# jiali-ms/JLM

Measured on AMD Instinct MI355X. Metric: decoded chars/sec at beam=10, vocab=50k (kana strings in -> n-best strings out, SURVEY 8d), higher is better.
Workload: dtype f32 (matrix products as 3-pass split-f16 MFMA, f32 accumulate; the vocabulary projection as f16 hi.hi + both cross terms in one block-scaled FP6 instruction per 32 k-values: f32-grade error, tests/test_gpu_kernels.py; scores f64; parity bars: step logits <= 1e-4 relative, 1-best identical, path scor

## Files before the change

__graft_entry__.py:

```python
import os
import subprocess
import sys

REPO = os.path.dirname(os.path.abspath(__file__))
CSRC = os.path.join(REPO, "jlm_amd", "csrc")
HIP_SOURCES = ["jlm_gemm.hip", "jlm_beam.hip", "jlm_split.hip", "jlm_gate.hip", "jlm_gate_p2.hip", "jlm_mixed.hip", "jlm_decode.hip", "jlm_score.hip", "jlm_topk.hip", "jlm_kmeans.hip", "jlm_train.hip"]
HOST_SOURCES = ["jlm_lattice.cpp"]


def _stale(target, sources):
    if not os.path.exists(target):
        return True
    t = os.path.getmtime(target)
    import glob
    deps = list(sources) + glob.glob(os.path.join(CSRC, "*.h")) + glob.glob(os.path.join(REPO, "include", "*.h"))
    return any(os.path.exists(s) and os.path.getmtime(s) > t for s in deps)


def _hipcc_accepts(hipcc, flags):
    key = (hipcc, tuple(flags))
    if key not in _hipcc_accepts.cache:
        import tempfile
        with tempfile.TemporaryDirectory() as d:
            src = os.path.join(d, "probe.hip")
            with open(src, "w") as f:
                f.write("__global__ void probe_kernel(float *p) { p[0] = 1.0f; }\n")
            rc = subprocess.call([hipcc, "--offload-arch=gfx950", "-c", "--cuda-device-only", "-o", os.path.join(d, "probe.o")] + list(flags) + [src],
                                 stdout=subprocess.DEVNULL, stderr=subprocess.DEVNULL)
        _hipcc_accepts.cache[key] = rc == 0
    return _hipcc_accepts.cache[key]


_hipcc_accepts.cache = {}


def build(force=False):
    hipcc = os.environ.get("HIPCC", "/opt/rocm/bin/hipcc")
    out = os.path.join(CSRC, "libjlm_hip.so")
    srcs = [os.path.join(CSRC, s) for s in HIP_SOURCES]
    if not _hipcc_accepts(hipcc, ["-mllvm", "-amdgpu-mfma-vgpr-form"]):
        raise RuntimeError("this hipcc does not accept -mllvm -amdgpu-mfma-vgpr-form: jlm_gate_ws.hip / jlm_mixed_w.hip cannot be built "
                           "correctly without it (their inline-asm loads into accumulation registers are not tracked by the compiler)")
    vgpr_form = ["-mllvm", "-amdgpu-mfma-vgpr-form"]
    no_nan = ["-fno-honor-nans", "-mno-amdgpu-ieee"]
    flagged = {"jlm_gate_ws.hip": vgpr_form, "jlm_mixed_w.hip": vgpr_form, "jlm_mx6.hip": no_nan + ["-fno-slp-vectorize"], "jlm_mx6w.hip": vgpr_form + no_nan,
               "jlm_frame_tail.hip": ["-fno-slp-vectorize"]}
    srcs = srcs + [os.path.join(CSRC, f) for f in flagged]
    if force or _stale(out, srcs):
        procs, objs = [], []
        for src in srcs:
            obj = src[:-4] + ".o"
            objs.append(obj)
            if force or _stale(obj, [src]):
                procs.append((src, subprocess.Popen([hipcc, "--offload-arch=gfx950", "-O3", "-std=c++17", "-fPIC", "-c", "-o", obj] +
                                                    flagged.get(os.path.basename(src), []) + [src], cwd=CSRC)))
        for src, pr in procs:
            if pr.wait() != 0:
                raise subprocess.CalledProcessError(pr.returncode, "hipcc -c " + src)
        subprocess.check_call([hipcc, "--offload-arch=gfx950", "-fPIC", "-shared", "-o", out] + objs, cwd=CSRC)
    host_srcs = [os.path.join(CSRC, s) for s in HOST_SOURCES if os.path.exists(os.path.join(CSRC, s))]
    if host_srcs:
        hout = os.path.join(CSRC, "libjlm_host.so")
        if force or _stale(hout, host_srcs):
            subprocess.check_call(["g++", "-O3", "-std=c++17", "-fPIC", "-shared", "-pthread", "-o", hout] + host_srcs,
                                  cwd=CSRC)
    rsrc = os.path.join(CSRC, "jlm_readout.c")
    rout = os.path.join(REPO, "jlm_amd", "_readout.so")
    if force or _stale(rout, [rsrc]):
        import sysconfig
        subprocess.check_call(["gcc", "-O2", "-fPIC", "-shared", "-I" + sysconfig.get_paths()["include"], "-o", rout, rsrc],
                              cwd=CSRC)
    tsrc = os.path.join(CSRC, "jlm_torch_ops.cpp")
    tout = os.path.join(REPO, "jlm_amd", "_torch_ops.so")
    if force or _stale(tout, [tsrc, out]):
        import torch
        from torch.utils import cpp_extension as ce
        tlib = ce.library_paths()[0]
        cmd = ["g++", "-O2", "-std=c++17", "-fPIC", "-shared", "-D__HIP_PLATFORM_AMD__", "-DUSE_ROCM",
               "-D_GLIBCXX_USE_CXX11_ABI=%d" % int(torch._C._GLIBCXX_USE_CXX11_ABI)]
        cmd += ["-I" + p for p in ce.include_paths()] + ["-I/opt/rocm/include", tsrc, "-o", tout, "-L" + tlib, "-ltorch", "-ltorch_cpu",
                                                         "-lc10", "-lc10_hip", "-ltorch_hip", "-L" + CSRC, "-ljlm_hip",
                                                         "-Wl,-rpath,$ORIGIN/csrc", "-Wl,-rpath," + tlib]
        subprocess.check_call(cmd, cwd=CSRC)
    if REPO not in sys.path:
        sys.path.insert(0, REPO)
    import jlm_amd
    from jlm_amd import _readout
    from jlm_amd import _lib, ops
    _lib.lib()
    ops.backend()
    from oracle import jlm_oracle


def smoke():
    import tempfile
    import numpy as np
    build()
    import torch
    assert torch.cuda.is_available(), "smoke() needs a GPU"
    from jlm_amd import config as jconfig, ops, synth
    assert type(ops.backend()).__name__ == "HipOps", "smoke() checks the HIP path (jlm_amd.ops.set_backend is a test hook)"
    from jlm_amd.decoder import Decoder
    from jlm_amd.decoder_dynamic import DynamicDecoder
    from oracle import jlm_oracle as orc
    root = tempfile.mkdtemp(prefix="jlm_smoke_")
    _cfg, _lex, _rd, alphabet = synth.build_fixture(root, "wide-vtable")
    jconfig.set_root(root)
    sents = synth.make_ragged_sentences(6, 3, 12, seed=42, alphabet=alphabet)
    score_atol = lambda s: 1e-6 * (len(s) + 1) + 2e-6
    dec = Decoder(1)
    assert dec.model.dev.mixed_idx == [0, 1, 2] or os.environ.get("JLM_LSE_MIXED") == "0" or os.environ.get("JLM_PRECISION") == "f32"
    got = dec.decode_batch(sents, beam_width=5)
    ref = orc.OracleDecoder(root, 1)
    for s, g in zip(sents, got):
        want = ref.decode(s, beam_width=5)
        assert [w for _, w in g][0] == [w for _, w in want][0], (s, g[0], want[0])
        np.testing.assert_allclose([x for x, _ in g], [x for x, _ in want], rtol=0, atol=score_atol(s))
    root2 = tempfile.mkdtemp(prefix="jlm_smoke_")
    synth.build_fixture(root2, "small-tied")
    jconfig.set_root(root2)
    dd = DynamicDecoder(1)
    got = dd.decode_batch(sents, beam_width=5, vocab_select=True)
    ref = orc.OracleDynamicDecoder(root2, 1)
    for s, g in zip(sents, got):
        want = ref.decode(s, beam_width=5, vocab_select=True)
        assert [w for _, w in g][0] == [w for _, w in want][0], (s, g[0], want[0])
        np.testing.assert_allclose([x for x, _ in g], [x for x, _ in want], rtol=0, atol=score_atol(s))
    print("smoke ok: static (D-softmax*) and dynamic decode match the oracle on", len(sents), "sentences")


if __name__ == "__main__":
    build(force="--force" in sys.argv)
    if "--smoke" in sys.argv:
        smoke()
```

jlm_amd/csrc/jlm_beam.hip:

```cpp
#include "jlm_common.h"
#include <type_traits>
#include <stdlib.h>

#define WL_THREADS 256
#define WL_ROWS 16

template <int MODE>
__global__ __launch_bounds__(WL_THREADS) void wordlist_kernel(
    SegTable segs, const float *__restrict__ b2, const float *__restrict__ T, int ldt,
    const int *__restrict__ g0v, const int *__restrict__ cnt, const int *__restrict__ cnt_idx,
    const int *__restrict__ wl, const int *__restrict__ wl_w, const int *__restrict__ wl_off, const int *__restrict__ wl_idx,
    int wl_base, const int *__restrict__ wl_out, float *__restrict__ edge, float *__restrict__ run_max,
    double *__restrict__ run_sum, double *__restrict__ lse, int merge, int beam) {
    extern __shared__ __attribute__((aligned(16))) float sm[];
    const int j = blockIdx.x;
    const int nrows = min(cnt[cnt_idx[j]], beam);
    if (nrows <= 0) return;
    const int gbase = g0v[j];
    const int lid = wl_base + wl_idx[j];
    const int w0 = wl_off[lid], nw = wl_off[lid + 1] - w0;
    if (MODE == 0 && nw == 0) return;
    const int tid = threadIdx.x;
    float *red = sm + (size_t)WL_ROWS * ldt;
    const int sub = tid & 7, slot = tid >> 3;
// ... 91 lines not shown
                for (int off = 32; off >= 1; off >>= 1) {
                    float m2 = __shfl_xor(rm[r], off), s2 = __shfl_xor(rs[r], off);
                    lse_merge(rm[r], rs[r], m2, s2);
                }
            }
            const int wave = tid >> 6, lane = tid & 63;
            __syncthreads();
            if (lane == 0)
                for (int r = 0; r < WL_ROWS; ++r) {
                    red[(wave * WL_ROWS + r) * 2] = rm[r];
                    red[(wave * WL_ROWS + r) * 2 + 1] = rs[r];
                }
            __syncthreads();
            if (tid < WL_ROWS && rc + tid < nrows) {
                float m = red[tid * 2], s = red[tid * 2 + 1];
                for (int w2 = 1; w2 < WL_THREADS / 64; ++w2)
                    lse_merge(m, s, red[(w2 * WL_ROWS + tid) * 2], red[(w2 * WL_ROWS + tid) * 2 + 1]);
                const int g = gbase + rc + tid;
                double S = (double)s;
                float M = m;
                if (merge) {
                    const float pm = run_max[g];
                    const double ps = run_sum[g];
                    M = fmaxf(pm, m);
                    S = ps * exp((double)pm - (double)M) + (double)s * exp((double)m - (double)M);
                }
                run_max[g] = M;
                run_sum[g] = S;
                lse[g] = (double)M + log(S);
            }
        }
    }
}

static int seg_table(const jlm_segment *segs_host, int n_segs, SegTable &t) {
    if (n_segs < 1 || n_segs > JLM_MAX_SEGMENTS) return -1;
    t.n = n_segs;
    for (int i = 0; i < n_segs; ++i) {
        t.s[i] = segs_host[i];
        if (t.s[i].k % 4 || t.s[i].ldb % 4 || t.s[i].t_off % 4) return -1;
    }
    return 0;
}

static size_t wl_lds_bytes(int , int ldt) { return ((size_t)WL_ROWS * ldt + 4 * WL_ROWS * 2) * sizeof(float); }

extern "C" int jlm_edge_logits(const jlm_segment *segs_host, int n_segs, const float *b2, const float *T, int ldt,
                               const int *g0, const int *cnt, const int *cnt_idx, const int *wl, const int *wl_off,
                               const int *wl_idx, int wl_base, const int *wl_out, float *edge, int beam, int n_groups,
                               void *stream) {
    return jlm_edge_logits_perm(segs_host, n_segs, b2, T, ldt, g0, cnt, cnt_idx, wl, nullptr, wl_off, wl_idx, wl_base, wl_out,
                                edge, beam, n_groups, stream);
}

extern "C" int jlm_edge_logits_perm(const jlm_segment *segs_host, int n_segs, const float *b2, const float *T, int ldt,
                                    const int *g0, const int *cnt, const int *cnt_idx, const int *wl, const int *wl_w,
                                    const int *wl_off, const int *wl_idx, int wl_base, const int *wl_out, float *edge, int beam,
                                    int n_groups, void *stream) {
    SegTable t;
    if (seg_table(segs_host, n_segs, t) || ldt % 4) return -1;
    if (n_groups <= 0) return 0;
    size_t lds = wl_lds_bytes(beam, ldt);
    if (lds > 160 * 1024) return -1;
    static JlmLdsGrant grant;
    if (int rc = jlm_grant_lds(grant, reinterpret_cast<const void *>(wordlist_kernel<0>), (int)lds)) return rc;
    hipLaunchKernelGGL(wordlist_kernel<0>, dim3(n_groups), dim3(WL_THREADS), lds, (hipStream_t)stream, t, b2, T, ldt,
                       g0, cnt, cnt_idx, wl, wl_w, wl_off, wl_idx, wl_base, wl_out, edge, nullptr, nullptr, nullptr, 0, beam);
    JLM_LAUNCH_CHECK();
    return 0;
}

static bool wl_split_hosts(const jlm_segment &s, int ldt) {
    const int ns = (s.k + 15) / 16;
    return ns >= 1 && ns <= 16 && s.k % 4 == 0 && s.ldb % 16 == 0 && s.ldb >= ns * 16 && s.t_off % 4 == 0 && ldt % 4 == 0;
}

extern "C" int jlm_wordlist_lse_form(const jlm_segment *segs_host, int n_segs, const jlm_segment *split_seg, int has_wl_w, int ldt,
                                     int beam, int max_words) {
    if (split_seg && n_segs == 1 && !has_wl_w && beam <= 64 && max_words >= JLM_WL_SPLIT_MIN_WORDS &&
        max_words <= JLM_WL_SPLIT_MAX_WORDS && wl_split_hosts(*split_seg, ldt))
        return JLM_WL_SPLIT;
    SegTable t;
    if (seg_table(segs_host, n_segs, t) || ldt % 4) return -1;
    static int use_mfma = -1;
    if (use_mfma < 0) { const char *e = getenv("JLM_WORDLIST_MFMA"); use_mfma = e ? atoi(e) : 1; }
    if (!has_wl_w && use_mfma && n_segs == 1 && beam <= 64 && segs_host[0].k >= 1 && segs_host[0].k <= 256) return JLM_WL_MFMA;
    if (wl_lds_bytes(beam, ldt) > 160 * 1024) return -1;
    return JLM_WL_F32;
}

extern "C" int jlm_wordlist_merge_form(const jlm_segment *segs_host, int n_segs, const jlm_segment *split_seg, int ldt, int beam,
                                       int max_words) {
    if (split_seg && n_segs == 1 && beam <= 64 && max_words <= JLM_WL_MERGE_MAX_WORDS && wl_split_hosts(*split_seg, ldt))
        return JLM_WL_MERGE_SPLIT;
    return jlm_wordlist_lse_form(segs_host, n_segs, split_seg, 0, ldt, beam, max_words);
}

extern "C" int jlm_wordlist_lse_mfma(const jlm_segment *seg_host, const float *b2, const float *T, int ldt, const int *g0,
                                     const int *cnt, const int *cnt_idx, const int *wl, const int *wl_off,
                                     const int *wl_idx, int wl_base, float *run_max, double *run_sum, double *lse,
                                     int merge, int beam, int n_groups, void *stream);

extern "C" int jlm_wordlist_lse(const jlm_segment *segs_host, int n_segs, const float *b2, const float *T, int ldt,
                                const int *g0, const int *cnt, const int *cnt_idx, const int *wl, const int *wl_off,
                                const int *wl_idx, int wl_base, float *run_max, double *run_sum, double *lse, int merge,
                                int beam, int n_groups, void *stream) {
    return jlm_wordlist_lse_perm(segs_host, n_segs, b2, T, ldt, g0, cnt, cnt_idx, wl, nullptr, wl_off, wl_idx, wl_base, run_max,
                                 run_sum, lse, merge, beam, n_groups, stream);
}

extern "C" int jlm_wordlist_lse_perm(const jlm_segment *segs_host, int n_segs, const float *b2, const float *T, int ldt,
                                     const int *g0, const int *cnt, const int *cnt_idx, const int *wl, const int *wl_w,
                                     const int *wl_off, const int *wl_idx, int wl_base, float *run_max, double *run_sum,
                                     double *lse, int merge, int beam, int n_groups, void *stream) {
    SegTable t;
    if (seg_table(segs_host, n_segs, t) || ldt % 4) return -1;
    if (n_groups <= 0) return 0;
    const int form = jlm_wordlist_lse_form(segs_host, n_segs, nullptr, wl_w != nullptr, ldt, beam, 0);
    if (form < 0) return -1;
    if (form == JLM_WL_MFMA)
        return jlm_wordlist_lse_mfma(segs_host, b2, T, ldt, g0, cnt, cnt_idx, wl, wl_off, wl_idx, wl_base, run_max, run_sum,
                                     lse, merge, beam, n_groups, stream);
    const size_t lds = wl_lds_bytes(beam, ldt);
    static JlmLdsGrant grant;
    if (int rc = jlm_grant_lds(grant, reinterpret_cast<const void *>(wordlist_kernel<1>), (int)lds)) return rc;
    hipLaunchKernelGGL(wordlist_kernel<1>, dim3(n_groups), dim3(WL_THREADS), lds, (hipStream_t)stream, t, b2, T, ldt,
                       g0, cnt, cnt_idx, wl, wl_w, wl_off, wl_idx, wl_base, nullptr, nullptr, run_max, run_sum, lse, merge, beam);
    JLM_LAUNCH_CHECK();
    return 0;
}

template <int CTRL, int ROW_MASK>
__device__ __forceinline__ void argmin_dpp_step(double &v, int &i) {
    const int lo = __double2loint(v), hi = __double2hiint(v);
    const int lo2 = __builtin_amdgcn_update_dpp(lo, lo, CTRL, ROW_MASK, 0xf, false);
    const int hi2 = __builtin_amdgcn_update_dpp(hi, hi, CTRL, ROW_MASK, 0xf, false);
    const int i2 = __builtin_amdgcn_update_dpp(i, i, CTRL, ROW_MASK, 0xf, false);
    const double v2 = __hiloint2double(hi2, lo2);
    if (v2 < v || (v2 == v && i2 < i)) { v = v2; i = i2; }
}
__device__ __forceinline__ void wave_argmin(double &v, int &i) {
    argmin_dpp_step<0xB1, 0xf>(v, i);
    argmin_dpp_step<0x4E, 0xf>(v, i);
    argmin_dpp_step<0x141, 0xf>(v, i);
    argmin_dpp_step<0x140, 0xf>(v, i);
    argmin_dpp_step<0x142, 0xa>(v, i);
    argmin_dpp_step<0x143, 0xc>(v, i);
    const int lo = __builtin_amdgcn_readlane(__double2loint(v), 63);
    const int hi = __builtin_amdgcn_readlane(__double2hiint(v), 63);
    i = __builtin_amdgcn_readlane(i, 63);
    v = __hiloint2double(hi, lo);
}

template <int MODE>
__global__ __launch_bounds__(64, 8) void beam_step_kernel(jlm_lattice lat, jlm_beam_state st, int frame, int max_cands) {
    extern __shared__ __attribute__((aligned(16))) double keys[];
    const int s = blockIdx.x, lane = threadIdx.x;
    const int B = lat.n_sent, beam = lat.beam, rmax = B * beam;
    const int len = lat.sent_len[s];
    const int fs = frame * B + s;
    if (frame > len) { if (lane == 0) st.cnt[fs] = 0; return; }
    const int nb = lat.end_off[fs], ne = lat.end_off[fs + 1];
    const int gout = frame * rmax + s * beam;
    const double INF = __longlong_as_double(0x7ff0000000000000LL);
    double *Sarr = keys + max_cands;
    int *gp_of = reinterpret_cast<int *>(Sarr + (MODE == 2 ? lat.n_frames * beam : 0));
    double *lse_new = reinterpret_cast<double *>(gp_of + ((max_cands + 1) & ~1));
    int *cnt_s = reinterpret_cast<int *>(lse_new + beam);
    double *win_v = reinterpret_cast<double *>(cnt_s + ((lat.n_frames + 1) & ~1));
    int *win_i = reinterpret_cast<int *>(win_v + beam);
    int K;
    if (frame == 0) {
        K = 1;
    } else {
        const bool fused = MODE == 0 && st.lse_part != nullptr;
        const int fprev = (frame - 1) * B + s;
        for (int f = lane; f < frame; f += 64) cnt_s[f] = st.cnt[f * B + s];
        const int kprev = st.cnt[fprev];
        if (fused && kprev > 0) {
            const int base = st.live_base[fprev];
            const float2 *part = reinterpret_cast<const float2 *>(st.lse_part);
            const int sub = lane & 7;
            for (int r0 = 0; r0 < kprev; r0 += 8) {
                const int r = r0 + (lane >> 3);
                float m = JLM_NEG_BIG;
                double sm = 0.0;
                if (r < kprev)
                    for (int p = sub; p < st.n_parts; p += 8) {
                        const float2 v = part[(size_t)p * st.ld_part + base + r];
                        const float mm = fmaxf(m, v.x);
                        sm = sm * (double)expf(m - mm) + (double)v.y * (double)expf(v.x - mm);
                        m = mm;
                    }
#pragma unroll
                for (int off = 4; off >= 1; off >>= 1) {
                    const float m2 = __shfl_xor(m, off);
                    const double s2 = __shfl_xor(sm, off);
                    const float mm = fmaxf(m, m2);
                    sm = sm * (double)expf(m - mm) + s2 * (double)expf(m2 - mm);
                    m = mm;
                }
                if (sub == 0 && r < kprev) {
                    double l = (double)m + log(sm);
                    if (!(fabs(l) < 1.0e300)) { if (st.flags) atomicOr(st.flags, 1); l = 1.0e30; }
                    lse_new[r] = l;
                    st.lse[(size_t)(frame - 1) * rmax + s * beam + r] = l;
                }
            }
        }
        const int C = (ne - nb) * beam;
        if (MODE == 2) {
            for (int f = 0; f < frame; ++f) {
                const int c = st.cnt[f * B + s];
                for (int l = lane; l < c; l += 64) {
                    const int g = f * rmax + s * beam + l;
                    const int p = st.bp[g];
                    double S = 0.0;
                    if (p >= 0) {
                        const int pf = p / rmax, pk = p - pf * rmax - s * beam;
                        S = Sarr[pf * beam + pk] + st.lse[p];
                    }
                    Sarr[f * beam + l] = S;
                }
                __syncthreads();
            }
        }
        __syncthreads();
        int nvalid = 0;
        double bv = INF;
        int bi = 0x7fffffff;
        constexpr int U = 4, NREG = 8;
        double kreg[NREG];
#pragma unroll
        for (int j = 0; j < NREG; ++j) kreg[j] = INF;
        auto group = [&](int it, auto REG0) {
            constexpr int reg0 = decltype(REG0)::value;
            const int c0 = lane + 64 * U * it;
            int n[U], k[U], sf[U];
#pragma unroll
            for (int u = 0; u < U; ++u) {
                const int c = min(c0 + 64 * u, C - 1);
                n[u] = nb + c / beam;
                k[u] = c % beam;
                sf[u] = lat.node_start[n[u]];
            }
            bool ok[U];
            double scv[U], lsv[U], ysv[U];
            float ev[U];
#pragma unroll
            for (int u = 0; u < U; ++u) {
                ok[u] = (c0 + 64 * u < C) && k[u] < cnt_s[sf[u]];
                const int gp = sf[u] * rmax + s * beam + (ok[u] ? k[u] : 0);
                ev[u] = st.edge[(size_t)n[u] * beam + k[u]];
                scv[u] = (MODE == 2) ? 0.0 : st.score[gp];
                lsv[u] = (MODE == 1) ? 0.0 : st.lse[gp];
                ysv[u] = (MODE == 2) ? st.ysum[gp] : 0.0;
                if (c0 + 64 * u < C) gp_of[c0 + 64 * u] = ok[u] ? gp : -1;
            }
#pragma unroll
            for (int u = 0; u < U; ++u) {
                const int c = c0 + 64 * u;
                if (c >= C) break;
                double sc = INF;
                if (ok[u]) {
                    const double e = (double)ev[u];
                    if (MODE == 0) sc = scv[u] + (((fused && sf[u] == frame - 1) ? lse_new[k[u]] : lsv[u]) - e);
                    else if (MODE == 1) sc = scv[u] - e;
                    else sc = (Sarr[sf[u] * beam + k[u]] + lsv[u]) - (ysv[u] + e);
                    ++nvalid;
                }
                if constexpr (reg0 >= 0) kreg[reg0 + u] = sc; else keys[c] = sc;
                if (sc < bv) { bv = sc; bi = c; }
            }
        };
        group(0, std::integral_constant<int, 0>{});
        if (C > 64 * U) group(1, std::integral_constant<int, U>{});
        for (int it = 2; 64 * U * it < C; ++it) group(it, std::integral_constant<int, -1>{});
#pragma unroll
        for (int off = 32; off >= 1; off >>= 1) nvalid += __shfl_xor(nvalid, off);
        K = min(beam, nvalid);
        for (int r = 0; r < K; ++r) {
            double v = bv;
            int i = bi;
            wave_argmin(v, i);
            if (lane == 0) { win_v[r] = v; win_i[r] = i; }
            if ((i & 63) == lane) {
                const int jw = i >> 6;
                if (jw >= NREG) keys[i] = INF;
                bv = INF;
                bi = 0x7fffffff;
#pragma unroll
                for (int j = 0; j < NREG; ++j) {
                    if (j == jw) kreg[j] = INF;
                    if (kreg[j] < bv) { bv = kreg[j]; bi = lane + 64 * j; }
                }
                for (int c = lane + 64 * NREG; c < C; c += 64) {
                    const double kv = keys[c];
                    if (kv < bv) { bv = kv; bi = c; }
                }
            }
        }
        __syncthreads();
    }
    for (int r = lane; r < K; r += 64) {
        const int g = gout + r;
        if (frame == 0) {
            st.score[g] = 0.0;
            if (st.ysum) st.ysum[g] = 0.0;
            st.bp[g] = -1;
            st.node[g] = nb;
            st.word[g] = lat.node_word[nb];
        } else {
            const int wi = win_i[r];
            const int n = nb + wi / beam, k = wi % beam;
            const int gp = gp_of[wi];
            st.score[g] = win_v[r];
            if (MODE == 2) st.ysum[g] = st.ysum[gp] + (double)st.edge[(size_t)n * beam + k];
            st.bp[g] = gp;
            st.node[g] = n;
            st.word[g] = lat.node_word[n];
        }
    }
    int base = 0;
    if (lane == 0) {
        st.cnt[fs] = K;
        if (frame < len) {
            base = atomicAdd(&st.n_live[frame], K);
            if (st.live_base) st.live_base[fs] = base;
        }
    }
    base = __shfl(base, 0);
    if (frame < len)
        for (int r = lane; r < K; r += 64) st.live[(size_t)frame * rmax + base + r] = gout + r;
}

template <int MODE>
__global__ __launch_bounds__(64) void beam_step_chunked_kernel(jlm_lattice lat, jlm_beam_state st, int frame, int cap, int nch_max) {
    extern __shared__ __attribute__((aligned(16))) double keys[];
    const int s = blockIdx.x, lane = threadIdx.x;
    const int B = lat.n_sent, beam = lat.beam, rmax = B * beam;
    const int len = lat.sent_len[s];
    const int fs = frame * B + s;
    if (frame > len) { if (lane == 0) st.cnt[fs] = 0; return; }
    const int nb = lat.end_off[fs], ne = lat.end_off[fs + 1];
    const int gout = frame * rmax + s * beam;
    const double INF = __longlong_as_double(0x7ff0000000000000LL);
    double *Sarr = keys + cap;
    int *gp_of = reinterpret_cast<int *>(Sarr + (MODE == 2 ? lat.n_frames * beam : 0));
    double *lse_new = reinterpret_cast<double *>(gp_of + ((cap + 1) & ~1));
    int *cnt_s = reinterpret_cast<int *>(lse_new + beam);
    double *win_v = reinterpret_cast<double *>(cnt_s + ((lat.n_frames + 1) & ~1));
    int *win_i = reinterpret_cast<int *>(win_v + beam);
    int *win_g = win_i + beam;
    double *cw_v = reinterpret_cast<double *>(win_g + beam + (beam & 1));
    int *cw_i = reinterpret_cast<int *>(cw_v + (size_t)nch_max * beam);
    int *cw_g = cw_i + (size_t)nch_max * beam;
    int K;
    if (frame == 0) {
        K = 1;
    } else {
        const bool fused = MODE == 0 && st.lse_part != nullptr;
        const int fprev = (frame - 1) * B + s;
        for (int f = lane; f < frame; f += 64) cnt_s[f] = st.cnt[f * B + s];
        const int kprev = st.cnt[fprev];
        if (fused && kprev > 0) {
            const int base = st.live_base[fprev];
            const float2 *part = reinterpret_cast<const float2 *>(st.lse_part);
            const int sub = lane & 7;
            for (int r0 = 0; r0 < kprev; r0 += 8) {
                const int r = r0 + (lane >> 3);
                float m = JLM_NEG_BIG;
                double sm = 0.0;
                if (r < kprev)
                    for (int p = sub; p < st.n_parts; p += 8) {
                        const float2 v = part[(size_t)p * st.ld_part + base + r];
                        const float mm = fmaxf(m, v.x);
                        sm = sm * (double)expf(m - mm) + (double)v.y * (double)expf(v.x - mm);
                        m = mm;
                    }
#pragma unroll
                for (int off = 4; off >= 1; off >>= 1) {
                    const float m2 = __shfl_xor(m, off);
                    const double s2 = __shfl_xor(sm, off);
                    const float mm = fmaxf(m, m2);
                    sm = sm * (double)expf(m - mm) + s2 * (double)expf(m2 - mm);
                    m = mm;
                }
                if (sub == 0 && r < kprev) {
                    double l = (double)m + log(sm);
                    if (!(fabs(l) < 1.0e300)) { if (st.flags) atomicOr(st.flags, 1); l = 1.0e30; }
                    lse_new[r] = l;
                    st.lse[(size_t)(frame - 1) * rmax + s * beam + r] = l;
                }
            }
        }
        const int C = (ne - nb) * beam;
        if (MODE == 2) {
            for (int f = 0; f < frame; ++f) {
                const int c = st.cnt[f * B + s];
                for (int l = lane; l < c; l += 64) {
                    const int g = f * rmax + s * beam + l;
                    const int p = st.bp[g];
                    double S = 0.0;
                    if (p >= 0) {
                        const int pf = p / rmax, pk = p - pf * rmax - s * beam;
                        S = Sarr[pf * beam + pk] + st.lse[p];
                    }
                    Sarr[f * beam + l] = S;
                }
                __syncthreads();
            }
        }
        __syncthreads();
        const int nch = (C + cap - 1) / cap;
        int nvalid_all = 0;
        for (int ch = 0; ch < nch; ++ch) {
            const int c_lo = ch * cap, Cc = min(C - c_lo, cap);
            int nvalid = 0;
            double bv = INF;
            int bi = 0x7fffffff;
            for (int lc = lane; lc < Cc; lc += 64) {
                const int c = c_lo + lc;
                const int n = nb + c / beam, k = c % beam;
                const int sf = lat.node_start[n];
                const bool ok = k < cnt_s[sf];
                const int gp = sf * rmax + s * beam + (ok ? k : 0);
                double sc = INF;
                if (ok) {
                    const double e = (double)st.edge[(size_t)n * beam + k];
                    if (MODE == 0) sc = st.score[gp] + (((fused && sf == frame - 1) ? lse_new[k] : st.lse[gp]) - e);
                    else if (MODE == 1) sc = st.score[gp] - e;
                    else sc = (Sarr[sf * beam + k] + st.lse[gp]) - (st.ysum[gp] + e);
                    ++nvalid;
                }
                keys[lc] = sc;
                gp_of[lc] = ok ? gp : -1;
                if (sc < bv) { bv = sc; bi = lc; }
            }
#pragma unroll
            for (int off = 32; off >= 1; off >>= 1) nvalid += __shfl_xor(nvalid, off);
            nvalid_all += nvalid;
            const int Kc = min(beam, nvalid);
            __syncthreads();
            for (int r = 0; r < beam; ++r) {
                if (r < Kc) {
                    double v = bv;
                    int i = bi;
                    wave_argmin(v, i);
                    if (lane == 0) { cw_v[ch * beam + r] = v; cw_i[ch * beam + r] = c_lo + i; cw_g[ch * beam + r] = gp_of[i]; }
                    if ((i & 63) == lane) {
                        keys[i] = INF;
                        bv = INF;
                        bi = 0x7fffffff;
                        for (int lc = lane; lc < Cc; lc += 64) {
                            const double kv = keys[lc];
                            if (kv < bv) { bv = kv; bi = lc; }
                        }
                    }
                } else if (lane == 0) {
                    cw_v[ch * beam + r] = INF; cw_i[ch * beam + r] = 0x7fffffff; cw_g[ch * beam + r] = -1;
                }
            }
            __syncthreads();
        }
        K = min(beam, nvalid_all);
        const int E = nch * beam;
        double bv = INF;
        int bi = 0x7fffffff, be = -1;
        for (int e = lane; e < E; e += 64) {
            const double v = cw_v[e];
            const int i = cw_i[e];
            if (v < bv || (v == bv && i < bi)) { bv = v; bi = i; be = e; }
        }
        for (int r = 0; r < K; ++r) {
            double v = bv;
            int i = bi;
            wave_argmin(v, i);
            if (bi == i && be >= 0) {
                win_v[r] = v; win_i[r] = i; win_g[r] = cw_g[be];
                cw_v[be] = INF; cw_i[be] = 0x7fffffff;
                bv = INF; bi = 0x7fffffff; be = -1;
                for (int e = lane; e < E; e += 64) {
                    const double v2 = cw_v[e];
                    const int i2 = cw_i[e];
                    if (v2 < bv || (v2 == bv && i2 < bi)) { bv = v2; bi = i2; be = e; }
                }
            }
        }
        __syncthreads();
    }
    for (int r = lane; r < K; r += 64) {
        const int g = gout + r;
        if (frame == 0) {
            st.score[g] = 0.0;
            if (st.ysum) st.ysum[g] = 0.0;
            st.bp[g] = -1;
            st.node[g] = nb;
            st.word[g] = lat.node_word[nb];
        } else {
            const int wi = win_i[r];
            const int n = nb + wi / beam, k = wi % beam;
            const int gp = win_g[r];
            st.score[g] = win_v[r];
            if (MODE == 2) st.ysum[g] = st.ysum[gp] + (double)st.edge[(size_t)n * beam + k];
            st.bp[g] = gp;
            st.node[g] = n;
            st.word[g] = lat.node_word[n];
        }
    }
    int base = 0;
    if (lane == 0) {
        st.cnt[fs] = K;
        if (frame < len) {
            base = atomicAdd(&st.n_live[frame], K);
            if (st.live_base) st.live_base[fs] = base;
        }
    }
    base = __shfl(base, 0);
    if (frame < len)
        for (int r = lane; r < K; r += 64) st.live[(size_t)frame * rmax + base + r] = gout + r;
}

static size_t beam_step_lds_bytes(int beam, int n_frames, int mode, int max_cands) {
    return (size_t)max_cands * sizeof(double) + (mode == 2 ? (size_t)n_frames * beam * sizeof(double) : 0) +
           (size_t)((max_cands + 1) & ~1) * sizeof(int) + (size_t)beam * sizeof(double) + (size_t)((n_frames + 1) & ~1) * sizeof(int) +
           (size_t)beam * (sizeof(double) + sizeof(int)) + 8;
}

static size_t beam_step_chunked_lds_bytes(int beam, int n_frames, int mode, int cap, int nch) {
    return beam_step_lds_bytes(beam, n_frames, mode, cap) + (size_t)(beam + (beam & 1)) * sizeof(int) +
           (size_t)nch * beam * (sizeof(double) + 2 * sizeof(int));
}
static int beam_step_chunk_cap(int beam, int n_frames, int mode) {
    const size_t fixed = beam_step_lds_bytes(beam, n_frames, mode, 0);
    if (fixed + 256 * 12 > 160 * 1024) return 0;
    size_t c = (160 * 1024 - fixed) / 12 / 2;
    return (int)(c / 256 * 256);
}
static int beam_step_one_chunk_max(int beam, int n_frames, int mode) {
    const size_t fixed = beam_step_lds_bytes(beam, n_frames, mode, 0);
    if (fixed + 256 * 12 > 160 * 1024) return 0;
    size_t c = (160 * 1024 - fixed) / 12;
    c = c / 256 * 256;
    while (c > 0 && beam_step_lds_bytes(beam, n_frames, mode, (int)c) > 160 * 1024) c -= 256;
    return (int)c;
}

extern "C" int jlm_beam_step_max_cands(int beam, int n_frames, int mode) {
    if (beam < 1 || beam > JLM_MAX_BEAM || n_frames < 1 || mode < 0 || mode > 2) return 0;
    const int one = beam_step_one_chunk_max(beam, n_frames, mode);
    const int cap = beam_step_chunk_cap(beam, n_frames, mode);
    if (one <= 0) return 0;
    if (cap <= 0) return one;
    const size_t base = beam_step_chunked_lds_bytes(beam, n_frames, mode, cap, 0);
    if (base >= 160 * 1024) return one;
    const size_t nch = (160 * 1024 - base) / ((size_t)beam * 16);
    size_t total = nch * (size_t)cap;
    if (total > (1u << 22)) total = 1u << 22;
    total = total / 256 * 256;
    return total > (size_t)one ? (int)total : one;
}

extern "C" int jlm_beam_step_lds_bytes(int beam, int n_frames, int mode, int max_cands) {
    if (beam < 1 || beam > JLM_MAX_BEAM || n_frames < 1 || mode < 0 || mode > 2 || max_cands < 1 || max_cands > (1 << 22)) return 0;
    return (int)beam_step_lds_bytes(beam, n_frames, mode, max_cands);
}

extern "C" int jlm_beam_step(const jlm_lattice *lat_host, const jlm_beam_state *st_host, int frame, int mode,
                             int max_cands, void *stream) {
    const jlm_lattice lat = *lat_host;
    const jlm_beam_state st = *st_host;
    if (lat.n_sent <= 0) return 0;
    if (mode == 2 && !st.ysum) return -1;
    if (mode < 0 || mode > 2) return -1;
    if (lat.beam < 1 || lat.beam > JLM_MAX_BEAM) return -1;
    if (st.lse_part && (!st.live_base || st.n_parts < 1 || mode != 0)) return -1;
    if (max_cands < 1) max_cands = 1;
    const size_t lds = beam_step_lds_bytes(lat.beam, lat.n_frames, mode, max_cands);
    static const int chunk_env = getenv("JLM_BEAM_CHUNK") ? atoi(getenv("JLM_BEAM_CHUNK")) : 0;
    if (lds > 160 * 1024 || chunk_env > 0) {
        const int cap = chunk_env > 0 ? chunk_env : beam_step_chunk_cap(lat.beam, lat.n_frames, mode);
        if (cap <= 0) return -1;
        const int nch = (max_cands + cap - 1) / cap;
        const size_t lds_c = beam_step_chunked_lds_bytes(lat.beam, lat.n_frames, mode, cap, nch);
        if (lds_c > 160 * 1024) return -1;
        const void *fc = mode == 0 ? (const void *)beam_step_chunked_kernel<0>
                       : mode == 1 ? (const void *)beam_step_chunked_kernel<1> : (const void *)beam_step_chunked_kernel<2>;
        static JlmLdsGrant grant_c[3];
        if (lds_c > 64 * 1024)
            if (int rc = jlm_grant_lds(grant_c[mode], fc, (int)lds_c)) return rc;
        if (mode == 0) hipLaunchKernelGGL(beam_step_chunked_kernel<0>, dim3(lat.n_sent), dim3(64), lds_c, (hipStream_t)stream, lat, st, frame, cap, nch);
        else if (mode == 1) hipLaunchKernelGGL(beam_step_chunked_kernel<1>, dim3(lat.n_sent), dim3(64), lds_c, (hipStream_t)stream, lat, st, frame, cap, nch);
        else hipLaunchKernelGGL(beam_step_chunked_kernel<2>, dim3(lat.n_sent), dim3(64), lds_c, (hipStream_t)stream, lat, st, frame, cap, nch);
        JLM_LAUNCH_CHECK();
        return 0;
    }
    const void *fn = mode == 0 ? (const void *)beam_step_kernel<0>
                   : mode == 1 ? (const void *)beam_step_kernel<1> : (const void *)beam_step_kernel<2>;
    static JlmLdsGrant grant[3];
    if (lds > 64 * 1024)
        if (int rc = jlm_grant_lds(grant[mode], fn, (int)lds)) return rc;
    if (mode == 0) hipLaunchKernelGGL(beam_step_kernel<0>, dim3(lat.n_sent), dim3(64), lds, (hipStream_t)stream, lat, st, frame, max_cands);
    else if (mode == 1) hipLaunchKernelGGL(beam_step_kernel<1>, dim3(lat.n_sent), dim3(64), lds, (hipStream_t)stream, lat, st, frame, max_cands);
    else hipLaunchKernelGGL(beam_step_kernel<2>, dim3(lat.n_sent), dim3(64), lds, (hipStream_t)stream, lat, st, frame, max_cands);
    JLM_LAUNCH_CHECK();
    return 0;
}

__global__ void backtrace_kernel(jlm_lattice lat, jlm_beam_state st, int *out_nodes, int *out_len, double *out_score,
                                 int stride) {
    const int idx = blockIdx.x * blockDim.x + threadIdx.x;
    const int B = lat.n_sent, beam = lat.beam, rmax = B * beam;
    if (idx >= rmax) return;
    const int s = idx / beam, r = idx % beam;
    const int len = lat.sent_len[s];
    const int c = st.cnt[len * B + s];
    if (r >= c) { out_len[idx] = 0; out_score[idx] = 0.0; return; }
    int g = len * rmax + s * beam + r;
    out_score[idx] = st.score[g];
    int d = 0;
    while (g >= 0 && d < stride) {
        out_nodes[(size_t)idx * stride + d] = st.node[g];
        ++d;
        g = st.bp[g];
    }
    out_len[idx] = d;
}

template <int NREG>
__global__ __launch_bounds__(64) void backtrace_wave_kernel(jlm_lattice lat, jlm_beam_state st, int *out_nodes, int *out_len, double *out_score,
                                                            int stride) {
    const int s = blockIdx.x, lane = threadIdx.x;
    const int B = lat.n_sent, beam = lat.beam, rmax = B * beam;
    const int len = lat.sent_len[s];
    const int E = (len + 1) * beam;
    int nd[NREG], pl[NREG];
#pragma unroll
    for (int j = 0; j < NREG; ++j) {
        const int e = lane + 64 * j;
        const int f = e / beam, k = e - f * beam;
        const bool in = e < E;
        const size_t g = (size_t)(in ? f : 0) * rmax + s * beam + (in ? k : 0);
        const int n = st.node[g], p = st.bp[g];
        nd[j] = in ? n : -1;
        int q = -1;
        if (in && p >= 0) { const int pf = p / rmax; q = pf * beam + (p - pf * rmax - s * beam); }
        pl[j] = q;
    }
    const int c = st.cnt[len * B + s];
    const bool valid = lane < beam && lane < c;
    const int idx = s * beam + lane;
    int e = valid ? len * beam + lane : -1, d = 0;
    const int steps = min(stride, len + 1);
    for (int t = 0; t < steps; ++t) {
        const int src = e & 63, jr = e >> 6;
        int nv = -1, pv = -1;
#pragma unroll
        for (int j = 0; j < NREG; ++j) {
            const int a = __shfl(nd[j], src), b2 = __shfl(pl[j], src);
            if (jr == j) { nv = a; pv = b2; }
        }
        if (e >= 0) {
            out_nodes[(size_t)idx * stride + d] = nv;
            ++d;
            e = pv;
        }
    }
    if (lane < beam) {
        out_len[idx] = valid ? d : 0;
        out_score[idx] = valid ? st.score[(size_t)len * rmax + s * beam + lane] : 0.0;
    }
}

extern "C" int jlm_backtrace(const jlm_lattice *lat_host, const jlm_beam_state *st_host, int *out_nodes, int *out_len,
                             double *out_score, int stride, void *stream) {
    const jlm_lattice lat = *lat_host;
    const jlm_beam_state st = *st_host;
    const int total = lat.n_sent * lat.beam;
    if (total <= 0) return 0;
// ... 60 lines not shown
```

Before: 3.063 million.

## Restructure beam step kernel to hoist loads and overlap LSE fold with candidate gather

Rewrites the per-frame beam step kernel so that the scalar header values (sentence length, end offsets, previous count, live base) are fetched in one parallel load across lanes. The LSE partial-fold loads for the first rows and the node start/word gathers for the first 512 candidates are now issued up front and parked in LDS, so their latencies overlap. Candidate indices are stepped incrementally instead of computed with per-element division, and in MODE 2 the back-pointer prefix setup is precomputed in LDS. The live-slot atomic is moved earlier, and the beam file is built with the atomic optimizer disabled. In exchange the kernel uses more registers and LDS, and the code is considerably harder to follow.

Result: no change. 3.063 million, median of 2 (-0.0%).

```diff
diff --git a/__graft_entry__.py b/__graft_entry__.py
--- a/__graft_entry__.py
+++ b/__graft_entry__.py
@@ -44,8 +44,9 @@
     vgpr_form = ["-mllvm", "-amdgpu-mfma-vgpr-form"]
     no_nan = ["-fno-honor-nans", "-mno-amdgpu-ieee"]
     flagged = {"jlm_gate_ws.hip": vgpr_form, "jlm_mixed_w.hip": vgpr_form, "jlm_mx6.hip": no_nan + ["-fno-slp-vectorize"], "jlm_mx6w.hip": vgpr_form + no_nan,
-               "jlm_frame_tail.hip": ["-fno-slp-vectorize"]}
-    srcs = srcs + [os.path.join(CSRC, f) for f in flagged]
+               "jlm_frame_tail.hip": ["-fno-slp-vectorize"],
+               "jlm_beam.hip": ["-mllvm", "-amdgpu-atomic-optimizer-strategy=None"]}
+    srcs = srcs + [os.path.join(CSRC, f) for f in flagged if f not in HIP_SOURCES]
     if force or _stale(out, srcs):
         procs, objs = [], []
         for src in srcs:
diff --git a/jlm_amd/csrc/jlm_beam.hip b/jlm_amd/csrc/jlm_beam.hip
--- a/jlm_amd/csrc/jlm_beam.hip
+++ b/jlm_amd/csrc/jlm_beam.hip
@@ -267,133 +267,319 @@
     v = __hiloint2double(hi, lo);
 }
 
+#define BS_PREV_ROWS 1024
+__device__ __forceinline__ void bs_advance(int &nrel, int &k, int d64, int r64, int beam) {
+    nrel += d64;
+    k += r64;
+    if (k >= beam) { k -= beam; ++nrel; }
+}
+__device__ __forceinline__ void fold_load4(const float2 *__restrict__ part, int ld_part, int n_parts, int row, int p0, float2 (&v)[4]) {
+#pragma unroll
+    for (int i = 0; i < 4; ++i) v[i] = part[(size_t)min(p0 + 8 * i, n_parts - 1) * ld_part + row];
+}
+__device__ __forceinline__ void fold_eat4(const float2 (&v)[4], int n_parts, int p0, bool row_ok, float &m, double &sm) {
+#pragma unroll
+    for (int i = 0; i < 4; ++i)
+        if (row_ok && p0 + 8 * i < n_parts) {
+            const float mm = fmaxf(m, v[i].x);
+            sm = sm * (double)expf(m - mm) + (double)v[i].y * (double)expf(v[i].x - mm);
+            m = mm;
+        }
+}
+__device__ __forceinline__ void fold_lanes(float &m, double &sm) {
+#pragma unroll
+    for (int off = 4; off >= 1; off >>= 1) {
+        const float m2 = __shfl_xor(m, off);
+        const double s2 = __shfl_xor(sm, off);
+        const float mm = fmaxf(m, m2);
+        sm = sm * (double)expf(m - mm) + s2 * (double)expf(m2 - mm);
+        m = mm;
+    }
+}
+
 template <int MODE>
 __global__ __launch_bounds__(64, 8) void beam_step_kernel(jlm_lattice lat, jlm_beam_state st, int frame, int max_cands) {
     extern __shared__ __attribute__((aligned(16))) double keys[];
     const int s = blockIdx.x, lane = threadIdx.x;
     const int B = lat.n_sent, beam = lat.beam, rmax = B * beam;
-    const int len = lat.sent_len[s];
-    const int fs = frame * B + s;
-    if (frame > len) { if (lane == 0) st.cnt[fs] = 0; return; }
-    const int nb = lat.end_off[fs], ne = lat.end_off[fs + 1];
+    const int fs = frame * B + s, fprev = fs - B;
+    const bool fused = MODE == 0 && st.lse_part != nullptr;
     const int gout = frame * rmax + s * beam;
     const double INF = __longlong_as_double(0x7ff0000000000000LL);
+    constexpr int U = 4, NREG = 8;
     double *Sarr = keys + max_cands;
     int *gp_of = reinterpret_cast<int *>(Sarr + (MODE == 2 ? lat.n_frames * beam : 0));
     double *lse_new = reinterpret_cast<double *>(gp_of + ((max_cands + 1) & ~1));
     int *cnt_s = reinterpret_cast<int *>(lse_new + beam);
     double *win_v = reinterpret_cast<double *>(cnt_s + ((lat.n_frames + 1) & ~1));
     int *win_i = reinterpret_cast<int *>(win_v + beam);
+    int *row_prev = win_i + beam;
+    int2 *park = reinterpret_cast<int2 *>(keys);
+
+    const int *p1 = lat.sent_len + s;
+    if (lane == 1) p1 = lat.end_off + fs;
+    if (lane == 2) p1 = lat.end_off + fs + 1;
+    if (frame > 0) {
+        if (lane == 3) p1 = st.cnt + fprev;
+        if (fused && lane == 4) p1 = st.live_base + fprev;
+    }
+    const int v1 = *p1;
+    int cf = 0;
+    if (lane < frame) cf = st.cnt[lane * B + s];
+    if (MODE == 2) {
+        const int R = frame * beam;
+        for (int e0 = 0; e0 < R; e0 += 64 * U) {
+            int pr[U];
+            double lr[U];
+#pragma unroll
+            for (int u = 0; u < U; ++u) {
+                const int e = min(e0 + lane + 64 * u, R - 1);
+                const int f = e / beam;
+                const size_t g = (size_t)f * rmax + s * beam + (e - f * beam);
+                pr[u] = st.bp[g];
+                lr[u] = st.lse[g];
+            }
+#pragma unroll
+            for (int u = 0; u < U; ++u) {
+                const int e = e0 + lane + 64 * u;
+                if (e < R) {
+                    const int p = pr[u];
+                    const int pf = p / rmax;
+                    if (e < BS_PREV_ROWS) row_prev[e] = p >= 0 ? pf * beam + (p - pf * rmax - s * beam) : -1;
+                    Sarr[e] = lr[u];
+                }
+            }
+        }
+    }
+    const int len = __builtin_amdgcn_readlane(v1, 0);
+    if (frame > len) { if (lane == 0) st.cnt[fs] = 0; return; }
+    const int nb = __builtin_amdgcn_readlane(v1, 1), ne = __builtin_amdgcn_readlane(v1, 2);
+    if (lane < frame) cnt_s[lane] = cf;
+    if (frame > 64) {
+        int lane_f = lane;
+        asm volatile("" : "+v"(lane_f));
+#pragma clang loop vectorize(disable) unroll(disable)
+        for (int f = lane_f + 64; f < frame; f += 64) cnt_s[f] = st.cnt[f * B + s];
+    }
+
+    int live_at = 0;
+    auto publish = [&](int K) {
+        if (lane == 0) {
+            st.cnt[fs] = K;
+            if (frame < len) live_at = atomicAdd(&st.n_live[frame], K);
+        }
+    };
     int K;
     if (frame == 0) {
         K = 1;
+        publish(K);
     } else {
-        const bool fused = MODE == 0 && st.lse_part != nullptr;
-        const int fprev = (frame - 1) * B + s;
-        for (int f = lane; f < frame; f += 64) cnt_s[f] = st.cnt[f * B + s];
-        const int kprev = st.cnt[fprev];
-        if (fused && kprev > 0) {
-            const int base = st.live_base[fprev];
-            const float2 *part = reinterpret_cast<const float2 *>(st.lse_part);
-            const int sub = lane & 7;
+        const int kprev = __builtin_amdgcn_readlane(v1, 3), base = __builtin_amdgcn_readlane(v1, 4);
+        const int C = (ne - nb) * beam;
+        const bool fold = fused && kprev > 0;
+        const int sub = lane & 7, rsub = lane >> 3;
+        const float2 *part = reinterpret_cast<const float2 *>(fold ? (const void *)st.lse_part : (const void *)lat.end_off);
+        const int ld_part = fold ? st.ld_part : 0, n_parts = fold ? st.n_parts : 1, row_base = fold ? base : 0, rows = fold ? kprev : 1;
+        float2 pv0[4], pv1[4];
+        fold_load4(part, ld_part, n_parts, row_base + min(rsub, rows - 1), sub, pv0);
+        fold_load4(part, ld_part, n_parts, row_base + min(8 + rsub, rows - 1), sub, pv1);
+        const int d64 = 64 / beam, r64 = 64 - d64 * beam;
+        const int nrel0 = lane / beam, k0 = lane - nrel0 * beam;
+        const int nlast = ne - nb - 1;
+        if (C > 0) {
+            int sf[NREG], wd[NREG];
+            int nrel = nrel0, k = k0, lane_a = lane;
+            asm volatile("" : "+v"(lane_a));
+#pragma unroll
+            for (int j = 0; j < NREG; ++j) {
+                const int n = nb + (lane_a + 64 * j < C ? nrel : nlast);
+                sf[j] = lat.node_start[n];
+                wd[j] = lat.node_word[n];
+                bs_advance(nrel, k, d64, r64, beam);
+            }
+#pragma unroll
+            for (int j = 0; j < NREG; ++j) park[min(lane_a + 64 * j, C - 1)] = make_int2(wd[j], sf[j]);
+        }
+#pragma unroll
+        for (int i = 0; i < 4; ++i) asm volatile("" : : "v"(pv0[i].x), "v"(pv0[i].y), "v"(pv1[i].x), "v"(pv1[i].y));
+        if (fold) {
             for (int r0 = 0; r0 < kprev; r0 += 8) {
-                const int r = r0 + (lane >> 3);
+                const int r = r0 + rsub;
+                const bool row_ok = r < kprev;
+                const int row = base + min(r, kprev - 1);
                 float m = JLM_NEG_BIG;
                 double sm = 0.0;
-                if (r < kprev)
-                    for (int p = sub; p < st.n_parts; p += 8) {
-                        const float2 v = part[(size_t)p * st.ld_part + base + r];
-                        const float mm = fmaxf(m, v.x);
-                        sm = sm * (double)expf(m - mm) + (double)v.y * (double)expf(v.x - mm);
-                        m = mm;
-                    }
-#pragma unroll
-                for (int off = 4; off >= 1; off >>= 1) {
-                    const float m2 = __shfl_xor(m, off);
-                    const double s2 = __shfl_xor(sm, off);
-                    const float mm = fmaxf(m, m2);
-                    sm = sm * (double)expf(m - mm) + s2 * (double)expf(m2 - mm);
-                    m = mm;
-                }
-                if (sub == 0 && r < kprev) {
-                    double l = (double)m + log(sm);
-                    if (!(fabs(l) < 1.0e300)) { if (st.flags) atomicOr(st.flags, 1); l = 1.0e30; }
-                    lse_new[r] = l;
-                    st.lse[(size_t)(frame - 1) * rmax + s * beam + r] = l;
-                }
-            }
-        }
-        const int C = (ne - nb) * beam;
-        if (MODE == 2) {
-            for (int f = 0; f < frame; ++f) {
-                const int c = st.cnt[f * B + s];
-                for (int l = lane; l < c; l += 64) {
-                    const int g = f * rmax + s * beam + l;
-                    const int p = st.bp[g];
-                    double S = 0.0;
-                    if (p >= 0) {
-                        const int pf = p / rmax, pk = p - pf * rmax - s * beam;
-                        S = Sarr[pf * beam + pk] + st.lse[p];
-                    }
-                    Sarr[f * beam + l] = S;
-                }
-                __syncthreads();
-            }
-        }
+                for (int pb = 0; pb < n_parts; pb += 32) {
+                    float2 v[4];
+                    if (pb > 0 || r0 >= 16) {
+                        fold_load4(part, ld_part, n_parts, row, pb + sub, v);
+                    } else {
+#pragma unroll
+                        for (int i = 0; i < 4; ++i) v[i] = r0 ? pv1[i] : pv0[i];
+                    }
+                    fold_eat4(v, n_parts, pb + sub, row_ok, m, sm);
+                }
+                fold_lanes(m, sm);
+                if (sub == 0 && row_ok) { win_v[r] = sm; win_i[r] = __float_as_int(m); }
+            }
+            __syncthreads();
+            for (int r = lane; r < kprev; r += 64) {
+                double l = (double)__int_as_float(win_i[r]) + log(win_v[r]);
+                if (!(fabs(l) < 1.0e300)) { if (st.flags) atomicOr(st.flags, 1); l = 1.0e30; }
+                lse_new[r] = l;
+            }
+        }
+        auto store_lse = [&]() {
+            if (fold)
+                for (int r = lane; r < kprev; r += 64) st.lse[(size_t)(frame - 1) * rmax + s * beam + r] = lse_new[r];
+        };
         __syncthreads();
         int nvalid = 0;
         double bv = INF;
         int bi = 0x7fffffff;
-        constexpr int U = 4, NREG = 8;
         double kreg[NREG];
 #pragma unroll
         for (int j = 0; j < NREG; ++j) kreg[j] = INF;
-        auto group = [&](int it, auto REG0) {
-            constexpr int reg0 = decltype(REG0)::value;
-            const int c0 = lane + 64 * U * it;
-            int n[U], k[U], sf[U];
-#pragma unroll
-            for (int u = 0; u < U; ++u) {
-                const int c = min(c0 + 64 * u, C - 1);
-                n[u] = nb + c / beam;
-                k[u] = c % beam;
-                sf[u] = lat.node_start[n[u]];
-            }
-            bool ok[U];
-            double scv[U], lsv[U], ysv[U];
-            float ev[U];
-#pragma unroll
-            for (int u = 0; u < U; ++u) {
-                ok[u] = (c0 + 64 * u < C) && k[u] < cnt_s[sf[u]];
-                const int gp = sf[u] * rmax + s * beam + (ok[u] ? k[u] : 0);
-                ev[u] = st.edge[(size_t)n[u] * beam + k[u]];
-                scv[u] = (MODE == 2) ? 0.0 : st.score[gp];
-                lsv[u] = (MODE == 1) ? 0.0 : st.lse[gp];
-                ysv[u] = (MODE == 2) ? st.ysum[gp] : 0.0;
-                if (c0 + 64 * u < C) gp_of[c0 + 64 * u] = ok[u] ? gp : -1;
-            }
-#pragma unroll
-            for (int u = 0; u < U; ++u) {
-                const int c = c0 + 64 * u;
-                if (c >= C) break;
-                double sc = INF;
-                if (ok[u]) {
-                    const double e = (double)ev[u];
-                    if (MODE == 0) sc = scv[u] + (((fused && sf[u] == frame - 1) ? lse_new[k[u]] : lsv[u]) - e);
-                    else if (MODE == 1) sc = scv[u] - e;
-                    else sc = (Sarr[sf[u] * beam + k[u]] + lsv[u]) - (ysv[u] + e);
-                    ++nvalid;
-                }
-                if constexpr (reg0 >= 0) kreg[reg0 + u] = sc; else keys[c] = sc;
+        auto count = [&]() {
+#pragma unroll
+            for (int off = 32; off >= 1; off >>= 1) nvalid += __shfl_xor(nvalid, off);
+            K = __builtin_amdgcn_readfirstlane(min(beam, nvalid));
+        };
+        const int gprev0 = (frame - 1) * rmax + s * beam;
+        if (C > 0) {
+            float ev[NREG];
+            double av[NREG], lv[NREG];
+            int nrel = nrel0, k = k0, lane_b = lane;
+            asm volatile("" : "+v"(nrel), "+v"(k), "+v"(lane_b));
+            int sfj[NREG];
+#pragma unroll
+            for (int j = 0; j < NREG; ++j) sfj[j] = park[min(lane_b + 64 * j, C - 1)].y;
+            unsigned okm = 0, pvm = 0;
+#pragma unroll
+            for (int j = 0; j < NREG; ++j) {
+                const int c = lane_b + 64 * j;
+                const bool in = c < C;
+                const int nr = in ? nrel : nlast, kk = in ? k : beam - 1;
+                const bool ok = in && kk < cnt_s[sfj[j]];
+                const int gp = sfj[j] * rmax + s * beam + (ok ? kk : 0);
+                ev[j] = st.edge[(size_t)(nb + nr) * beam + kk];
+                av[j] = (MODE == 2) ? st.ysum[gp] : st.score[gp];
+                lv[j] = (MODE == 0) ? st.lse[gp] : 0.0;
+                okm |= (unsigned)ok << j;
+                pvm |= (unsigned)(ok && sfj[j] == frame - 1) << j;
+                if (in) {
+                    gp_of[c] = ok ? gp : -1;
+                    if (MODE == 2) park[c].y = sfj[j] * beam + kk;
+                }
+                bs_advance(nrel, k, d64, r64, beam);
+            }
+            nvalid = __popc(okm);
+            store_lse();
+            if (C <= 64 * NREG) count();
+            if (MODE == 2) {
+                for (int f = 0; f < frame; ++f) {
+                    const int c = cnt_s[f];
+                    for (int l = lane; l < c; l += 64) {
+                        const int e = f * beam + l;
+                        int q;
+                        if (e < BS_PREV_ROWS) {
+                            q = row_prev[e];
+                        } else {
+                            const int p = st.bp[(size_t)f * rmax + s * beam + l];
+                            const int pf = p / rmax;
+                            q = p >= 0 ? pf * beam + (p - pf * rmax - s * beam) : -1;
+                        }
+                        double S = 0.0;
+                        if (q >= 0) S = Sarr[q];
+                        Sarr[e] = S + Sarr[e];
+                    }
+                    __syncthreads();
+                }
+            }
+            int lane_c = lane, kc = k0, nc = nrel0;
+            asm volatile("" : "+v"(lane_c), "+v"(kc), "+v"(nc));
+#pragma unroll
+            for (int j = 0; j < NREG; ++j) {
+                const int c = lane_c + 64 * j;
+                const bool ok = (okm >> j) & 1;
+                const double e = (double)ev[j];
+                double sc;
+                if (MODE == 0) {
+                    const bool prev = fused && ((pvm >> j) & 1);
+                    double ln = lse_new[prev ? kc : 0];
+                    asm volatile("" : "+v"(ln));
+                    sc = av[j] + ((prev ? ln : lv[j]) - e);
+                } else if (MODE == 1) {
+                    sc = av[j] - e;
+                } else {
+                    const int q = park[min(c, C - 1)].y;
+                    sc = Sarr[q] - (av[j] + e);
+                }
+                sc = ok ? sc : INF;
+                kreg[j] = sc;
                 if (sc < bv) { bv = sc; bi = c; }
-            }
-        };
-        group(0, std::integral_constant<int, 0>{});
-        if (C > 64 * U) group(1, std::integral_constant<int, U>{});
-        for (int it = 2; 64 * U * it < C; ++it) group(it, std::integral_constant<int, -1>{});
-#pragma unroll
-        for (int off = 32; off >= 1; off >>= 1) nvalid += __shfl_xor(nvalid, off);
-        K = min(beam, nvalid);
+                bs_advance(nc, kc, d64, r64, beam);
+            }
+            if (C > 64 * NREG) {
+                auto first_level = [&](int c0, int nrel_, int k_, int (&out)[U]) {
+#pragma unroll
+                    for (int u = 0; u < U; ++u) {
+                        out[u] = lat.node_start[nb + (c0 + 64 * u < C ? nrel_ : nlast)];
+                        bs_advance(nrel_, k_, d64, r64, beam);
+                    }
+                };
+                int sfn[U];
+                first_level(lane + 64 * NREG, nrel, k, sfn);
+                for (int c0 = lane + 64 * NREG; c0 - lane < C; c0 += 64 * U) {
+                    float eu[U];
+                    double au[U], lu[U];
+                    int qu[U];
+#pragma unroll
+                    for (int u = 0; u < U; ++u) {
+                        const int c = c0 + 64 * u;
+                        const bool in = c < C;
+                        const int nr = in ? nrel : nlast, kk = in ? k : beam - 1;
+                        const bool ok = in && kk < cnt_s[sfn[u]];
+                        const int gp = sfn[u] * rmax + s * beam + (ok ? kk : 0);
+                        eu[u] = st.edge[(size_t)(nb + nr) * beam + kk];
+                        au[u] = (MODE == 2) ? st.ysum[gp] : st.score[gp];
+                        lu[u] = (MODE == 0) ? st.lse[gp] : 0.0;
+                        qu[u] = (MODE == 2) ? sfn[u] * beam + kk : 0;
+                        if (in) gp_of[c] = ok ? gp : -1;
+                        nvalid += ok;
+                        bs_advance(nrel, k, d64, r64, beam);
+                    }
+                    if (c0 - lane + 64 * U < C) first_level(c0 + 64 * U, nrel, k, sfn);
+#pragma unroll
+                    for (int u = 0; u < U; ++u) {
+                        const int c = c0 + 64 * u;
+                        const int gp = gp_of[min(c, C - 1)];
+                        const bool ok = c < C && gp >= 0;
+                        const double e = (double)eu[u];
+                        double sc;
+                        if (MODE == 0) {
+                            const int kk = gp - gprev0;
+                            const bool prev = fused && ok && kk >= 0;
+                            double ln = lse_new[prev ? kk : 0];
+                            asm volatile("" : "+v"(ln));
+                            sc = au[u] + ((prev ? ln : lu[u]) - e);
+                        } else if (MODE == 1) {
+                            sc = au[u] - e;
+                        } else {
+                            sc = Sarr[qu[u]] - (au[u] + e);
+                        }
+                        sc = ok ? sc : INF;
+                        if (c < C) keys[c] = sc;
+                        if (sc < bv) { bv = sc; bi = c; }
+                    }
+                }
+                count();
+            }
+        } else {
+            store_lse();
+            K = 0;
+        }
+        publish(K);
         for (int r = 0; r < K; ++r) {
             double v = bv;
             int i = bi;
@@ -420,33 +606,30 @@
     for (int r = lane; r < K; r += 64) {
         const int g = gout + r;
         if (frame == 0) {
+            const int w = lat.node_word[nb];
             st.score[g] = 0.0;
             if (st.ysum) st.ysum[g] = 0.0;
             st.bp[g] = -1;
             st.node[g] = nb;
-            st.word[g] = lat.node_word[nb];
+            st.word[g] = w;
         } else {
             const int wi = win_i[r];
             const int n = nb + wi / beam, k = wi % beam;
             const int gp = gp_of[wi];
+            const int w = wi < 64 * NREG ? park[wi].x : lat.node_word[n];
+            double ys = 0.0;
+            if (MODE == 2) ys = st.ysum[gp] + (double)st.edge[(size_t)n * beam + k];
             st.score[g] = win_v[r];
-            if (MODE == 2) st.ysum[g] = st.ysum[gp] + (double)st.edge[(size_t)n * beam + k];
+            if (MODE == 2) st.ysum[g] = ys;
             st.bp[g] = gp;
             st.node[g] = n;
-            st.word[g] = lat.node_word[n];
-        }
-    }
-    int base = 0;
-    if (lane == 0) {
-        st.cnt[fs] = K;
-        if (frame < len) {
-            base = atomicAdd(&st.n_live[frame], K);
-            if (st.live_base) st.live_base[fs] = base;
-        }
-    }
-    base = __shfl(base, 0);
+            st.word[g] = w;
+        }
+    }
+    const int live0 = __builtin_amdgcn_readfirstlane(live_at);
+    if (lane == 0 && frame < len && st.live_base) st.live_base[fs] = live0;
     if (frame < len)
-        for (int r = lane; r < K; r += 64) st.live[(size_t)frame * rmax + base + r] = gout + r;
+        for (int r = lane; r < K; r += 64) st.live[(size_t)frame * rmax + live0 + r] = gout + r;
 }
 
 template <int MODE>
@@ -639,7 +822,8 @@
 static size_t beam_step_lds_bytes(int beam, int n_frames, int mode, int max_cands) {
     return (size_t)max_cands * sizeof(double) + (mode == 2 ? (size_t)n_frames * beam * sizeof(double) : 0) +
            (size_t)((max_cands + 1) & ~1) * sizeof(int) + (size_t)beam * sizeof(double) + (size_t)((n_frames + 1) & ~1) * sizeof(int) +
-           (size_t)beam * (sizeof(double) + sizeof(int)) + 8;
+           (size_t)beam * (sizeof(double) + sizeof(int)) + 8 +
+           (mode == 2 ? (size_t)(n_frames * beam < BS_PREV_ROWS ? n_frames * beam : BS_PREV_ROWS) * sizeof(int) : 0);
 }
 
 static size_t beam_step_chunked_lds_bytes(int beam, int n_frames, int mode, int cap, int nch) {
```
